# dkarpushkin/rs-pathtracing

Measured on AMD Instinct MI355X. Metric: Msamples/sec cornell_box 1920x1080x256spp at 1/2/4/8 MI355X; RMS pixel delta, higher is better.
Workload: dtype f64; 1 GPU; cornell_box.json 1920x1080 256spp depth 8; config=c2, width=1920, height=1080, spp=256, depth=8, seed=1, parallelism=single GPU, wf_slots=2

## Files before the change

rs-pathtracing_amd/csrc/pt_device.hpp:

```cpp
#pragma once
#include <hip/hip_runtime.h>

#include <cstdint>

#include "pt_lprof.hpp"
#include "pt_march.hpp"
#include "pt_torus.hpp"
#include "pt_types.hpp"

namespace pt {
namespace dev {

__device__ __forceinline__ bool stopped(const int *flag) {
    return flag && __hip_atomic_load(flag, __ATOMIC_RELAXED, __HIP_MEMORY_SCOPE_SYSTEM) != 0;
}

struct V3 {
    double x, y, z;
};
PT_HD V3 v3(double x, double y, double z) { return V3{x, y, z}; }
PT_HD V3 add(V3 a, V3 b) { return v3(a.x + b.x, a.y + b.y, a.z + b.z); }
PT_HD V3 sub(V3 a, V3 b) { return v3(a.x - b.x, a.y - b.y, a.z - b.z); }
PT_HD double dot(V3 a, V3 b) { return a.x * b.x + a.y * b.y + a.z * b.z; }
PT_HD V3 scale(V3 a, double s) { return v3(a.x * s, a.y * s, a.z * s); }
// ... 514 lines not shown
    default: {
        double g[3];
        march::shape_gradient_k<FK>(shape_params(s), p.x, p.y, p.z, g);
        n = v3(g[0], g[1], g[2]);
        break;
    }
    }
    n = normalize(n);
    V3 wn = xf_normal(s.inv, n);
    Hit h;
    h.front = dot(wn, r.d) < 0.0;
    h.n = normalize(h.front ? wn : neg(wn));
    h.p = xf_point(s.dir, p);
    return h;
}

PT_HD void hit_uv(const DShape &s, const Ray &r, double t, double *u, double *v) {
    V3 o = xf_point(s.inv, r.o);
    V3 d = xf_vector(s.inv, r.d);
    V3 p = v3(o.x + d.x * t, o.y + d.y * t, o.z + d.z * t);
    const double PI = 3.141592653589793;
    switch (s.type) {
    case SPHERE: {
        const double theta = acos(-p.y);
        const double phi = atan2(-p.z, p.x) + PI;
        *u = phi / (2.0 * PI);
        *v = theta / PI;
        return;
    }
    case RECTANGLE:
        *u = (p.x - s.p[0]) / (s.p[2] - s.p[0]);
        *v = (p.y - s.p[1]) / (s.p[3] - s.p[1]);
        return;
    case CUBE: {
        double ax = fabs(p.x), ay = fabs(p.y), az = fabs(p.z);
        double mc = fmax(fmax(ax, ay), az);
        if (mc == ax) *u = p.y, *v = p.z;
        else if (mc == ay) *u = p.x, *v = p.z;
        else if (mc == az) *u = p.x, *v = p.y;
        else *u = *v = __builtin_nan("");
        return;
    }
    case TORUS: {
        const double theta = asin(p.z / s.p[1]);
        const double phi = acos(p.z / (s.p[0] + s.p[1] * cos(theta))) + PI;
        *u = phi / (2.0 * PI);
        *v = theta / PI;
        return;
    }
    default:
        if (s.func == march::F_DUPIN || s.func == march::F_HUNTS || s.func == march::F_CUSHION) *u = p.x, *v = p.y;
        else *u = *v = 0.0;
        return;
    }
}

PT_HD int32_t sat_i32(double x) {
    if (!(x == x)) return 0;
    if (x >= 2147483647.0) return 2147483647;
    if (x <= -2147483648.0) return -2147483647 - 1;
    return (int32_t)x;
}
PT_HD uint32_t sat_u32(double x) {
    if (!(x > 0.0)) return 0u;
    if (x >= 4294967295.0) return 4294967295u;
    return (uint32_t)x;
}

PT_HD double perlin_noise(const DPerlin &P, V3 p) {
    const double fx = floor(p.x), fy = floor(p.y), fz = floor(p.z);
    const uint32_t x = (uint32_t)sat_i32(fx), y = (uint32_t)sat_i32(fy), z = (uint32_t)sat_i32(fz);
    const double u = p.x - fx, v = p.y - fy, w = p.z - fz;
    const double u2 = u * u * (3.0 - 2.0 * u);
    const double v2 = v * v * (3.0 - 2.0 * v);
    const double w2 = w * w * (3.0 - 2.0 * w);
    double acc = 0.0;
    for (int c = 0; c < 8; c++) {
        const int d0 = c >> 2, d1 = (c >> 1) & 1, d2 = c & 1;
        const int32_t k = P.perm[0][(x + (uint32_t)d0) & 255u] ^ P.perm[1][(y + (uint32_t)d1) & 255u] ^
                          P.perm[2][(z + (uint32_t)d2) & 255u];
        const double fi = (double)d0, fj = (double)d1, fk = (double)d2;
        const double dot = P.ranvec[k][0] * (u - fi) + P.ranvec[k][1] * (v - fj) + P.ranvec[k][2] * (w - fk);
        acc = acc + (fi * u2 + (double)(1 - d0) * (1.0 - u2)) * (fj * v2 + (double)(1 - d1) * (1.0 - v2)) *
                        (fk * w2 + (double)(1 - d2) * (1.0 - w2)) * dot;
    }
    return acc;
}
PT_HD double perlin_turb(const DPerlin &P, V3 p) {
    const double n = perlin_noise(P, p);
    double acc = 0.0, weight = 1.0;
    for (int i = 0; i < 7; i++) {
        acc = acc + weight * n;
        weight *= 0.5;
    }
    return fabs(acc);
}

PT_HD V3 tex_value(const Scene &sc, int node, double u, double v, V3 p) {
    const double PI = 3.141592653589793;
    for (int guard = 0; guard < 64; guard++) {
        const DTexture &t = sc.tex[node];
        switch (t.type) {
        case TEX_SOLID: return v3(t.c[0], t.c[1], t.c[2]);
        case TEX_CHECKER: {
            const double sines = sin(t.c[0] * p.x) * sin(t.c[1] * p.y) * sin(t.c[2] * p.z);
            node = sines < 0.0 ? t.odd : t.even;
            break;
        }
        case TEX_UVCHECKER: {
            const double sines = sin(v * t.c[0] * PI) * sin(u * t.c[1] * PI);
            node = sines < 0.0 ? t.odd : t.even;
            break;
        }
        case TEX_NOISE: {
            const double s = 0.5 * (1.0 + sin(t.c[0] * p.z + 10.0 * perlin_turb(sc.perlin[t.aux], p)));
            return v3(1.0 * s, 1.0 * s, 1.0 * s);
        }
        default: {
            const DImage im = sc.images[t.aux];
            const double uc = u < 0.0 ? 0.0 : (u > 1.0 ? 1.0 : u);
            const double vc = 1.0 - (v < 0.0 ? 0.0 : (v > 1.0 ? 1.0 : v));
            uint32_t x = sat_u32(uc * (double)im.width), y = sat_u32(vc * (double)im.height);
            x = x < im.width ? x : im.width - 1;
            y = y < im.height ? y : im.height - 1;
            const uint8_t *px = sc.pixels + im.offset + ((size_t)y * im.width + x) * 4;
            const double cs = 1.0 / 255.0;
            return v3((double)px[0] * cs, (double)px[1] * cs, (double)px[2] * cs);
        }
        }
    }
    return v3(__builtin_nan(""), __builtin_nan(""), __builtin_nan(""));
}

struct PhaseTimes {
    uint64_t trace, march, select, shade, passes, march_passes, finish, scatter, restart;
};
#if defined(__HIP_DEVICE_COMPILE__)
#define PT_STAMP() __builtin_amdgcn_s_memtime()
#else
#define PT_STAMP() 0ull
#endif

template <bool STATS = false>
PT_HD V3 random_in_unit_sphere(Rng &rng, double s11, Ctr *ct = nullptr) {
    for (;;) {
        PT_LP(REJECT_TRY);
        if (STATS) ct->c[C_REJECT_TRIES]++;
        double x = rng.uniform(-1.0, s11);
        double y = rng.uniform(-1.0, s11);
        double z = rng.uniform(-1.0, s11);
        if (x * x + y * y + z * z <= 1.0) return v3(x, y, z);
    }
}
PT_HD V3 reflect(V3 d, V3 n) {
    V3 b = scale(n, dot(d, n));
    return sub(d, scale(b, 2.0));
}
PT_HD V3 refract(V3 d, V3 n, double ratio) {
    double c = dot(neg(d), n);
    V3 perp = scale(add(d, scale(n, c)), ratio);
    double ps = -(sqrt(fabs(1.0 - dot(perp, perp))));
    return add(perp, scale(n, ps));
}
PT_HD V3 background(V3 d) {
    double t = 0.5 * (d.y + 1.0);
    double u = 1.0 * (1.0 - t);
    return v3(u + 0.5 * t, u + 0.7 * t, u + 1.0 * t);
}

constexpr uint32_t VAL_BIT = 0x80000000u;
template <int NW>
struct IdStack {
    uint64_t w[NW];
    int n;
    double *vb = nullptr;
    size_t vs = 0;
    PT_HD void push_val(V3 a) {
        vb[(size_t)(n * 3 + 0) * vs] = a.x;
        vb[(size_t)(n * 3 + 1) * vs] = a.y;
        vb[(size_t)(n * 3 + 2) * vs] = a.z;
        push(VAL_BIT);
    }
    PT_HD V3 val(int level) const {
        return v3(vb[(size_t)(level * 3 + 0) * vs], vb[(size_t)(level * 3 + 1) * vs], vb[(size_t)(level * 3 + 2) * vs]);
    }
    PT_HD void clear() {
#pragma unroll
        for (int i = 0; i < NW; i++) w[i] = 0;
        n = 0;
    }
    PT_HD void push(uint32_t id) {
#pragma unroll
        for (int i = NW - 1; i > 0; i--) w[i] = (w[i] << 32) | (w[i - 1] >> 32);
        w[0] = (w[0] << 32) | id;
        n++;
    }
    PT_HD uint32_t pop() {
        uint32_t id = (uint32_t)w[0];
#pragma unroll
        for (int i = 0; i < NW - 1; i++) w[i] = (w[i] >> 32) | (w[i + 1] << 32);
        w[NW - 1] >>= 32;
        n--;
        return id;
    }
};

PT_HD bool shade_decided(int who, uint32_t depth) { return depth == 0 || who < 0; }
PT_HD V3 decided_leaf(int who, const Ray &ray) { return who >= 0 ? v3(0.0, 0.0, 0.0) : background(ray.d); }

template <bool STATS = false, int FK = march::F_ANY, bool EXT = false, class Stack>
PT_HD bool shade(const Scene &sc, int who, double t, Ray &ray, uint32_t &depth, Stack &stk, Rng &rng,
                 double s11, V3 *leaf, Ctr *ct = nullptr, uint64_t *tfin = nullptr) {
    if (who < 0) {
        *leaf = background(ray.d);
        return true;
    }
    if (depth == 0) {
        *leaf = v3(0.0, 0.0, 0.0);
        return true;
    }
    const DShape &s = sc.shapes[who];
    if (STATS) ct->c[C_HITS]++;
    PT_LP(SHADE_HIT);
    Hit h = finish<FK>(s, ray, t);
    const DMaterial &m = sc.mats[s.material];
    if (tfin) *tfin = PT_STAMP();
    auto textured = [&]() {
        double u, v;
        hit_uv(s, ray, t, &u, &v);
        return tex_value(sc, m.tex, u, v, h.p);
    };
    V3 dir;
    if (m.type == LAMBERTIAN) {
        PT_LP(LAMBERT);
        if (STATS) ct->c[C_LAMBERT]++;
        V3 u = normalize(random_in_unit_sphere<STATS>(rng, s11, ct));
        dir = add(h.n, u);
        if (approx_zero(dir.x) && approx_zero(dir.y) && approx_zero(dir.z)) dir = h.n;
        if (EXT && m.tex >= 0) stk.push_val(textured());
        else stk.push((uint32_t)s.material);
    } else if (m.type == METAL) {
        PT_LP(METAL);
        if (STATS) ct->c[C_METAL]++;
        V3 rf = reflect(ray.d, h.n);
        dir = m.fuzz == 0.0 ? rf : add(rf, scale(random_in_unit_sphere<STATS>(rng, s11, ct), m.fuzz));
        if (EXT && m.tex >= 0) stk.push_val(textured());
        else stk.push((uint32_t)s.material);
    } else if (m.type == DIELECTRIC) {
        PT_LP(DIELECTRIC);
        if (STATS) ct->c[C_DIELECTRIC]++;
        double ratio = h.front ? 1.0 / m.ior : m.ior;
        double c = dot(neg(ray.d), h.n);
        double sn = sqrt(1.0 - c * c);
        bool refl = ratio * sn > 1.0;
        if (!refl) {
            double r0 = (1.0 - ratio) / (1.0 + ratio);
            r0 = r0 * r0;
            double x = 1.0 - c;
            double x5 = x * ((x * x) * (x * x));
            refl = r0 + (1.0 - r0) * x5 > rng.gen();
        }
        dir = refl ? reflect(ray.d, h.n) : refract(ray.d, h.n, ratio);
    } else {
        PT_LP(EMIT);
        if (EXT && m.type == DIFFUSE_LIGHT && m.tex >= 0) *leaf = textured();
        else *leaf = m.type == DIFFUSE_LIGHT ? v3(m.emit[0], m.emit[1], m.emit[2]) : v3(0.0, 0.0, 0.0);
        return true;
    }
    ray.o = h.p;
    ray.d = normalize(dir);
    depth--;
    return false;
}

template <bool STATS = false, bool EXT = false, class Stack>
PT_HD V3 unwind(const Scene &sc, Stack &stk, V3 c, Ctr *ct = nullptr) {
    while (stk.n > 0) {
        if (STATS) ct->c[C_UNWIND]++;
        const uint32_t id = stk.pop();
        if (EXT && (id & VAL_BIT)) {
            const V3 a = stk.val(stk.n);
            c = v3(a.x * c.x, a.y * c.y, a.z * c.z);
        } else {
            const DMaterial &m = sc.mats[id];
            c = v3(m.albedo[0] * c.x, m.albedo[1] * c.y, m.albedo[2] * c.z);
        }
    }
    return c;
}

struct MemStack {
    uint32_t *base;
    size_t stride;
    int n;
    double *vb;
    PT_HD void push_val(V3 a) {
        vb[(size_t)(n * 3 + 0) * stride] = a.x;
        vb[(size_t)(n * 3 + 1) * stride] = a.y;
        vb[(size_t)(n * 3 + 2) * stride] = a.z;
        push(VAL_BIT);
    }
    PT_HD V3 val(int level) const {
        return v3(vb[(size_t)(level * 3 + 0) * stride], vb[(size_t)(level * 3 + 1) * stride],
                  vb[(size_t)(level * 3 + 2) * stride]);
    }
    PT_HD void push(uint32_t id) {
        base[(size_t)n * stride] = id;
        n++;
    }
    PT_HD uint32_t pop() {
        n--;
        return base[(size_t)n * stride];
    }
};

template <bool EXT, class Stack>
PT_HD V3 ray_color_on(const Scene &sc, Ray ray, uint32_t depth, Rng &rng, double s11, Stack &stk) {
    V3 leaf;
    for (;;) {
        double t;
        const int who = closest<false, EXT>(sc, ray, T_MIN, __builtin_inf(), &t);
        if (shade<false, march::F_ANY, EXT>(sc, who, t, ray, depth, stk, rng, s11, &leaf)) break;
    }
    return unwind<false, EXT>(sc, stk, leaf);
}
template <int NW, bool EXT = false>
PT_HD V3 ray_color(const Scene &sc, Ray ray, uint32_t depth, Rng &rng, double s11, double *vb = nullptr,
                   size_t vs = 0) {
    IdStack<NW> stk;
    stk.clear();
    stk.vb = vb;
    stk.vs = vs;
    return ray_color_on<EXT>(sc, ray, depth, rng, s11, stk);
}
template <bool EXT = false>
PT_HD V3 ray_color_mem(const Scene &sc, Ray ray, uint32_t depth, Rng &rng, double s11, uint32_t *ids, double *vb,
                       size_t stride) {
    MemStack stk{ids, stride, 0, vb};
    return ray_color_on<EXT>(sc, ray, depth, rng, s11, stk);
}

PT_HD Ray camera_ray(const FrameParams &P, uint32_t x, uint32_t y, Rng &rng) {
    double u = rng.gen();
    double v = rng.gen();
    double sx = P.pixel_resolution * ((double)x + u);
    double sy = P.pixel_resolution * ((double)y + v);
    V3 d = v3((P.left_top[0] + P.right[0] * sx) - P.up[0] * sy, (P.left_top[1] + P.right[1] * sx) - P.up[1] * sy,
              (P.left_top[2] + P.right[2] * sx) - P.up[2] * sy);
    V3 pos = v3(P.pos[0], P.pos[1], P.pos[2]);
    Ray r;
    r.o = pos;
    r.d = normalize(sub(d, pos));
    return r;
}

constexpr int MARCH_ITERS = 2;

enum Phase : int { PH_TRACE = 0, PH_SELECT = 1, PH_MARCH = 2, PH_SHADE = 3 };


template <int NW, bool STATS = false, bool TIMING = false, int FK = march::F_ANY, bool EXT = false>
PT_HD V3 trace_pixel(const Scene &sc, const FrameParams &P, uint32_t x, uint32_t y, Ctr *ct = nullptr,
                     PhaseTimes *pt = nullptr, double *vb = nullptr, size_t vs = 0) {
    uint64_t pixel = (uint64_t)x + (uint64_t)y * P.width;
    V3 acc = v3(0.0, 0.0, 0.0);
    uint32_t s = 0;
    Rng rng{sample_key(P.seed, pixel, 0)};
    Ray ray = camera_ray(P, x, y, rng);
    uint32_t depth = P.depth;
    IdStack<NW> stk;
    stk.clear();
    stk.vb = vb;
    stk.vs = vs;
    const int nmarch = (sc.diag & 1) ? 0 : sc.nmarch;
    int phase = PH_TRACE, who = -1, km = 0, mshape = -1;
    double best = 0.0;
    V3 inv = v3(0.0, 0.0, 0.0);
    march::MarchState ms;
    march::MarchStats mst{0, 0, 0, 0};
    uint64_t ts = 0;
    for (;;) {
        if (TIMING) {
            ts = PT_STAMP();
            pt->passes++;
        }
        if (phase == PH_TRACE) {
            if (STATS) ct->c[C_BOUNCES]++;
            inv = v3(1.0 / ray.d.x, 1.0 / ray.d.y, 1.0 / ray.d.z);
            best = __builtin_inf();
            who = -1;
            closest_nomarch<STATS, EXT>(sc, ray, inv, T_MIN, &best, &who, ct);
            km = 0;
            phase = PH_SELECT;
        }
        if (TIMING) {
            uint64_t n = PT_STAMP();
            pt->trace += n - ts;
            ts = n;
// ... 83 lines not shown
```

rs-pathtracing_amd/csrc/pt_lprof.hpp:

```cpp
#pragma once
#include <hip/hip_runtime.h>

#ifdef PT_MARCH_REGIONS
namespace pt {
namespace mreg {
enum { R_ITER, R_POLY, R_PREFIX, R_HALVE, R_ADV, R_LIT, R_REFILL, R_TOTAL, R_N };
enum { P_iters, P_lin_init, P_lit_adds, P_advance_loops, P_evals, P_sir_inside, P_lin_fail_zero, P_lin_fail_q,
       P_lin_fail_tie, P_lin_fail_zone, P_N };
constexpr int G_N = 2 * R_N + 2 * P_N;
__device__ unsigned long long g_acc[G_N];
__shared__ unsigned long long t0[4][R_N], acc[4][R_N], accl[4][R_N], n0[4][R_N], pw[4][P_N], pl[4][P_N];
__device__ __forceinline__ unsigned long long now() {
    __builtin_amdgcn_sched_barrier(0);
    const unsigned long long t = __builtin_amdgcn_s_memtime();
    __builtin_amdgcn_sched_barrier(0);
    return t;
}
__device__ __forceinline__ bool leader() {
    const uint32_t lane = __builtin_amdgcn_mbcnt_hi(~0u, __builtin_amdgcn_mbcnt_lo(~0u, 0u));
    return lane == (uint32_t)__builtin_ctzll(__ballot(1));
}
__device__ __forceinline__ void begin(int r) {
    const unsigned long long m = __ballot(1);
    if (leader()) {
        t0[threadIdx.x >> 6][r] = now();
        n0[threadIdx.x >> 6][r] = __popcll(m);
    }
}
__device__ __forceinline__ void end(int r) {
    if (leader()) {
        const unsigned long long dt = now() - t0[threadIdx.x >> 6][r];
        acc[threadIdx.x >> 6][r] += dt;
        accl[threadIdx.x >> 6][r] += dt * n0[threadIdx.x >> 6][r];
    }
}
__device__ __forceinline__ void prof(int k) {
    const unsigned long long m = __ballot(1);
    if (leader()) {
        pw[threadIdx.x >> 6][k] += 1;
        pl[threadIdx.x >> 6][k] += __popcll(m);
    }
}
__device__ __forceinline__ void poly_begin() { begin(R_POLY); }
__device__ __forceinline__ void poly_end() { end(R_POLY); }
__device__ __forceinline__ void prefix_begin() { begin(R_PREFIX); }
__device__ __forceinline__ void prefix_end() { end(R_PREFIX); }
__device__ __forceinline__ void halve_begin() { begin(R_HALVE); }
__device__ __forceinline__ void halve_end() { end(R_HALVE); }
__device__ __forceinline__ void adv_begin() { begin(R_ADV); }
__device__ __forceinline__ void adv_end() { end(R_ADV); }
__device__ __forceinline__ void lit_begin() { begin(R_LIT); }
__device__ __forceinline__ void kernel_begin(unsigned long long *t_kernel) {
    if ((threadIdx.x & 63) == 0) {
        for (int k = 0; k < R_N; k++) t0[threadIdx.x >> 6][k] = acc[threadIdx.x >> 6][k] = accl[threadIdx.x >> 6][k] = 0;
        for (int k = 0; k < P_N; k++) pw[threadIdx.x >> 6][k] = pl[threadIdx.x >> 6][k] = 0;
    }
    *t_kernel = now();
}
__device__ __forceinline__ void step_end() {
    end(R_ITER);
    if (leader() && t0[threadIdx.x >> 6][R_LIT]) {
        const unsigned long long dt = now() - t0[threadIdx.x >> 6][R_LIT];
        acc[threadIdx.x >> 6][R_LIT] += dt;
        accl[threadIdx.x >> 6][R_LIT] += dt * n0[threadIdx.x >> 6][R_LIT];
        t0[threadIdx.x >> 6][R_LIT] = 0;
    }
}
__device__ __forceinline__ void kernel_end(unsigned long long t_kernel) {
    if ((threadIdx.x & 63) == 0) {
        const int w = threadIdx.x >> 6;
        acc[w][R_TOTAL] = now() - t_kernel;
        accl[w][R_TOTAL] = 0;
        for (int k = 0; k < R_N; k++) {
            atomicAdd(&g_acc[k], acc[w][k]);
            atomicAdd(&g_acc[R_N + k], accl[w][k]);
        }
        for (int k = 0; k < P_N; k++) {
            atomicAdd(&g_acc[2 * R_N + k], pw[w][k]);
            atomicAdd(&g_acc[2 * R_N + P_N + k], pl[w][k]);
        }
    }
}
}
}
#define PT_MREG(what) pt::mreg::what()
#define PT_MPROF(field) (pt::mreg::prof(pt::mreg::P_##field))
#define PT_MREG_KERNEL_BEGIN() \
    unsigned long long mreg_t_kernel_; \
    pt::mreg::kernel_begin(&mreg_t_kernel_)
#define PT_MREG_STEP_BEGIN() pt::mreg::begin(pt::mreg::R_ITER)
#define PT_MREG_STEP_END() pt::mreg::step_end()
#define PT_MREG_REFILL_BEGIN() pt::mreg::begin(pt::mreg::R_REFILL)
#define PT_MREG_REFILL_END() pt::mreg::end(pt::mreg::R_REFILL)
#define PT_MREG_KERNEL_END() pt::mreg::kernel_end(mreg_t_kernel_)
#else
#define PT_MREG_KERNEL_BEGIN() ((void)0)
#define PT_MREG_STEP_BEGIN() ((void)0)
#define PT_MREG_STEP_END() ((void)0)
#define PT_MREG_REFILL_BEGIN() ((void)0)
#define PT_MREG_REFILL_END() ((void)0)
#define PT_MREG_KERNEL_END() ((void)0)
#endif


namespace pt {
namespace lprof {
enum Point : int {
    LIVE,
    SHADE_HIT,
    LAMBERT,
    REJECT_TRY,
    METAL,
    DIELECTRIC,
    EMIT,
    ENDED,
    TRACE,
    ULIST_SHAPE,
    RECT_ROWS,
    UBOX_PASS,
    BVH_NODE,
    BVH_ENTER,
    BVH_LEAF,
    PRE_SLAB,
    PRE_JOB,
    ANY_END,
    MISS_END,
    STORE,
    N_POINTS
};
}
}

#if defined(PT_LANE_PROF)
namespace pt {
namespace lprof {
static __device__ unsigned long long g_counts[2 * N_POINTS];
static __shared__ unsigned long long s_pass[N_POINTS], s_lanes[N_POINTS];
__device__ __forceinline__ void hit(int k) {
    const unsigned long long m = __ballot(1);
    const uint32_t lane = __builtin_amdgcn_mbcnt_hi(~0u, __builtin_amdgcn_mbcnt_lo(~0u, 0u));
    if (lane == (uint32_t)__builtin_ctzll(m)) {
        atomicAdd(&s_pass[k], 1ull);
        atomicAdd(&s_lanes[k], (unsigned long long)__popcll(m));
    }
}
__device__ __forceinline__ void begin_kernel() {
    if (threadIdx.x < N_POINTS) s_pass[threadIdx.x] = s_lanes[threadIdx.x] = 0;
    __syncthreads();
}
__device__ __forceinline__ void end_kernel() {
    __syncthreads();
    if (threadIdx.x < N_POINTS) {
        atomicAdd(&g_counts[threadIdx.x], s_pass[threadIdx.x]);
        atomicAdd(&g_counts[N_POINTS + threadIdx.x], s_lanes[threadIdx.x]);
    }
}
}
}
#endif
#if defined(PT_LANE_PROF) && defined(__HIP_DEVICE_COMPILE__)
#define PT_LP(k) pt::lprof::hit(pt::lprof::k)
#define PT_LP_BEGIN() pt::lprof::begin_kernel()
#define PT_LP_END() pt::lprof::end_kernel()
#else
#define PT_LP(k) ((void)0)
#define PT_LP_BEGIN() ((void)0)
#define PT_LP_END() ((void)0)
#endif
```

rs-pathtracing_amd/csrc/pt_wave.hip:

```cpp
#include <hip/hip_runtime.h>

#include <cstdio>
#include <cstdlib>
#include <vector>

#include "pt_lprof.hpp"

#include "pt_device.hpp"
#include "pt_kernel.hpp"
#include "pt_plan.hpp"

namespace pt {

using dev::MemStack;
using dev::Ray;
using dev::V3;

constexpr uint32_t WHO_MASK = (1u << 25) - 1u;
__host__ __device__ __forceinline__ uint32_t pack_who(int who, uint32_t count) {
    return (uint32_t)(who + 1) | (count << 25);
}
__host__ __device__ __forceinline__ int unpack_who(uint32_t w) { return (int)(w & WHO_MASK) - 1; }

struct PathSoA {
    char *base;
    size_t cap;
    static constexpr size_t BYTES = PATH_BYTES;
    static constexpr uint32_t BLK = 64, BLK_BYTES = (uint32_t)BYTES * BLK;
    enum F8 : int { OX, OY, OZ, DX, DY, DZ, T, RNG };
    enum F4 : int { WHO, SID };
    __host__ __device__ double *d8(uint32_t k) const {
        return (double *)(base + (size_t)(k / BLK) * BLK_BYTES) + (k % BLK);
    }
    __host__ __device__ uint32_t *d4(uint32_t k) const {
        return (uint32_t *)(base + (size_t)(k / BLK) * BLK_BYTES + 8 * 8 * BLK) + (k % BLK);
    }
    __host__ __device__ double &t(uint32_t k) const { return d8(k)[T * BLK]; }
    __host__ __device__ uint32_t &who(uint32_t k) const { return d4(k)[WHO * BLK]; }
};

struct WfView {
    PathSoA in, out;
    uint32_t *ids;
    double *att;
    double *leaf;
    uint8_t *status;
    uint32_t *list, *mq;
    double2 *jo;
    uint32_t *cnt;
    double *acc;
    uint32_t cap;
    uint32_t npix;
    uint32_t s0, ns;
    uint32_t tile0;
};

struct WfArgs {
    dev::Scene sc;
    FrameParams P;
    WfView v;
};

template <class T>
__device__ __forceinline__ const T &kargs(const T *p) {
    typedef const __attribute__((address_space(4))) T *cptr;
    cptr q = (cptr)p;
    asm volatile("" : "+s"(q));
    return *(const T *)q;
}

__device__ __forceinline__ uint32_t lane_id() {
    return __builtin_amdgcn_mbcnt_hi(~0u, __builtin_amdgcn_mbcnt_lo(~0u, 0u));
}

constexpr int UB = 4;
template <bool EXT>
__device__ __forceinline__ V3 unwind_mem(const dev::Scene &sc, MemStack &stk, V3 c) {
    if (EXT) return dev::unwind<false, true>(sc, stk, c);
    while (stk.n > 0) {
        const int m = stk.n < UB ? stk.n : UB;
        uint32_t id[UB];
#pragma unroll
        for (int j = 0; j < UB; j++) id[j] = j < m ? stk.base[(size_t)(stk.n - 1 - j) * stk.stride] : 0u;
        double ax[UB], ay[UB], az[UB];
#pragma unroll
        for (int j = 0; j < UB; j++) {
            const DMaterial &mt = sc.mats[id[j]];
            ax[j] = j < m ? mt.albedo[0] : 1.0;
            ay[j] = j < m ? mt.albedo[1] : 1.0;
            az[j] = j < m ? mt.albedo[2] : 1.0;
        }
#pragma unroll
        for (int j = 0; j < UB; j++)
            if (j < m) c = dev::v3(ax[j] * c.x, ay[j] * c.y, az[j] * c.z);
        stk.n -= m;
    }
    return c;
}

__device__ __forceinline__ void end_path(const WfView &v, uint32_t id, const MemStack &stk, V3 leaf) {
    typedef double d2v __attribute__((ext_vector_type(2)));
    d2v *rec = (d2v *)(v.leaf + (size_t)id * 4);
    __builtin_nontemporal_store((d2v){leaf.x, leaf.y}, rec);
    __builtin_nontemporal_store((d2v){leaf.z, __builtin_bit_cast(double, (uint64_t)(uint32_t)stk.n)}, rec + 1);
}

template <typename T>
__device__ __forceinline__ void st_path(T *p, T x) {
    __builtin_nontemporal_store(x, p);
}
template <typename T>
__device__ __forceinline__ T ld_path(const T *p) {
    return *p;
}
__device__ __forceinline__ void store_path(const PathSoA &S, uint32_t k, uint32_t id, const Ray &ray, double best,
                                           int who, uint64_t rng, uint32_t count) {
    double *a = S.d8(k);
    uint32_t *b = S.d4(k);
    constexpr uint32_t B = PathSoA::BLK;
    st_path(a + PathSoA::OX * B, ray.o.x);
    st_path(a + PathSoA::OY * B, ray.o.y);
    st_path(a + PathSoA::OZ * B, ray.o.z);
    st_path(a + PathSoA::DX * B, ray.d.x);
    st_path(a + PathSoA::DY * B, ray.d.y);
    st_path(a + PathSoA::DZ * B, ray.d.z);
    st_path(a + PathSoA::T * B, best);
    st_path(b + PathSoA::WHO * B, pack_who(who, count));
    st_path((uint64_t *)a + PathSoA::RNG * B, (uint64_t)rng);
    st_path(b + PathSoA::SID * B, id);
}
__device__ __forceinline__ void load_path(const PathSoA &S, uint32_t p, uint32_t *id, Ray *ray, uint64_t *rng,
                                          uint32_t depth_it, uint32_t *depth, uint32_t *count, int *who,
                                          double *best) {
    const double *a = S.d8(p);
    const uint32_t *b = S.d4(p);
    constexpr uint32_t B = PathSoA::BLK;
    *id = ld_path(b + PathSoA::SID * B);
    ray->o = dev::v3(ld_path(a + PathSoA::OX * B), ld_path(a + PathSoA::OY * B), ld_path(a + PathSoA::OZ * B));
    ray->d = dev::v3(ld_path(a + PathSoA::DX * B), ld_path(a + PathSoA::DY * B), ld_path(a + PathSoA::DZ * B));
    *rng = ld_path((const uint64_t *)a + PathSoA::RNG * B);
    const uint32_t w = ld_path(b + PathSoA::WHO * B);
    *who = unpack_who(w);
    *count = w >> 25;
    *depth = depth_it;
    *best = ld_path(a + PathSoA::T * B);
}

static_assert(plan::PACKED_COUNT_DEPTH == MAX_REG_DEPTH, "the DEEP builds start where the register stacks end");
__device__ __forceinline__ uint32_t *deep_count(const WfView &v, uint32_t depth, uint32_t id) {
    return v.ids + (size_t)depth * v.cap + id;
}

__device__ __forceinline__ void slot_pixel(const FrameParams &P, const WfView &v, uint32_t id, uint32_t *x,
                                           uint32_t *y, uint32_t *s_local, uint32_t *pix_local) {
    const uint32_t within = id % v.npix;
    *s_local = id / v.npix;
    *pix_local = within;
    const uint32_t ti = v.tile0 + within / (TILE * TILE);
    const uint32_t th = within % (TILE * TILE);
    const uint32_t k = dev::tile_position(P.rank + ti * P.world, P.tiles_x, P.world);
    const uint32_t tx = k % P.tiles_x, ty = k / P.tiles_x;
    const uint32_t w = th >> 6, l = th & 63;
    *x = tx * TILE + (((w & 1u) << 3) | (l & 7u));
    *y = ty * TILE + (((w >> 1) << 3) | (l >> 3));
}

constexpr int WF_PREDICT = 4;

template <bool FIRST, int WAVES, int FK = march::F_ANY, bool EXT = false, bool BIGBVH = false, bool SPLIT = false,
          bool DEEP = false>
__global__ __launch_bounds__(256, WAVES) void wf_bounce(const WfArgs *__restrict__ A, int it,
                                                        unsigned long long *diag = nullptr) {
    uint32_t count;
    {
        const WfArgs &a = kargs(A);
        const WfView &v = a.v;
        count = FIRST ? (v.cnt[3] ? 0u : v.ns * v.npix) : v.cnt[it * 4 + 0];
        if (a.P.stop && blockIdx.x == 0 && threadIdx.x == 0 && v.cnt[3]) dev::note_stop(a.sc.guard, count > 0);
    }
    const uint32_t stride = gridDim.x * blockDim.x;
    const bool DIAG = PT_WAVE_DIAG && diag;
    unsigned long long dsec[7] = {0, 0, 0, 0, 0, 0, 0}, tst = 0;
    PT_LP_BEGIN();
#define PT_BSTAMP(k)                                                \
    if (DIAG) {                                                     \
        __builtin_amdgcn_s_waitcnt(0);                              \
        const unsigned long long n_ = __builtin_amdgcn_s_memtime(); \
        dsec[k] += n_ - tst;                                        \
        tst = n_;                                                   \
    }
    for (uint32_t base = blockIdx.x * blockDim.x; base < count; base += stride) {
        if (DIAG) tst = __builtin_amdgcn_s_memtime();
        const WfArgs &a = kargs(A);
        const dev::Scene &sc = a.sc;
        const FrameParams &P = a.P;
        const WfView &v = a.v;
        const uint32_t i = base + threadIdx.x;
        bool live = i < count;
        uint32_t id = 0;
        Ray ray;
        dev::Rng rng{0};
        uint32_t depth = 0;
        MemStack stk{v.ids, (size_t)v.cap, 0, nullptr};
        int who = -1;
        double best = 0.0;
        if (live) {
            if (FIRST) {
                id = i;
                uint32_t x, y, sl, pl;
                slot_pixel(P, v, id, &x, &y, &sl, &pl);
                if (x >= P.width || y >= P.height || sl >= v.ns) {
                    live = false;
                } else {
                    rng.s = dev::sample_key(P.seed, (uint64_t)x + (uint64_t)y * P.width, v.s0 + sl);
                    ray = dev::camera_ray(P, x, y, rng);
                    depth = P.depth;
                    stk.base = v.ids + id;
                    if (EXT) stk.vb = v.att + id;
                }
            } else {
                const uint32_t p = v.list[i];
                PT_BSTAMP(0)
                uint32_t count;
                load_path(v.in, p, &id, &ray, &rng.s, P.depth + 1u - (uint32_t)it, &depth, &count, &who, &best);
                stk.base = v.ids + id;
                stk.n = DEEP ? (int)*deep_count(v, P.depth, id) : (int)count;
                if (EXT) stk.vb = v.att + id;
                PT_BSTAMP(1)
            }
        }
        bool need_march = false, long_job = false;
        V3 jo_o = dev::v3(0.0, 0.0, 0.0), jo_d = jo_o;
        double jo_st = 0.0, jo_en = 0.0;
        if (live) {
            PT_LP(LIVE);
            if (!FIRST) {
                V3 leaf;
                const bool ended = dev::shade<false, FK, EXT>(kargs(A).sc, who, best, ray, depth, stk, rng, P.s11, &leaf);
                PT_BSTAMP(2)
                if (ended) {
                    PT_LP(ENDED);
                    end_path(v, id, stk, leaf);
                    live = false;
                    PT_BSTAMP(3)
                }
            }
        }
        if (live && SPLIT) {
            best = __builtin_inf();
            who = -1;
        } else if (live) {
            PT_LP(TRACE);
            const V3 inv = dev::v3(1.0 / ray.d.x, 1.0 / ray.d.y, 1.0 / ray.d.z);
            best = __builtin_inf();
            who = -1;
            const bool any = depth == 0;
            dev::closest_nomarch<false, EXT, BIGBVH>(kargs(A).sc, ray, inv, T_MIN, &best, &who, nullptr, any);
            PT_BSTAMP(4)
            for (int k = 0; k < sc.nmarch && !need_march && !(any && who >= 0); k++) {
                const int s = dev::uniform_index(dev::uniform_load(&sc.march[k]));
                const DBox bx = dev::uniform_box(&sc.boxes[s]);
                if (!dev::slab(bx.lo, bx.hi, ray, inv, T_MIN, best)) continue;
                PT_LP(PRE_SLAB);
                const DShape S = dev::uniform_shape(&sc.shapes[s]);
                jo_o = dev::xf_point(S.inv, ray.o);
                jo_d = dev::xf_vector(S.inv, ray.d);
                need_march = march::shape_bound_k<FK>(dev::shape_params(S), jo_o.x, jo_o.y, jo_o.z, jo_d.x, jo_d.y,
                                                      jo_d.z, &jo_st, &jo_en);
            }
            PT_BSTAMP(5)
            if (!need_march && dev::shade_decided(who, depth)) {
                if (any) PT_LP(ANY_END);
                else PT_LP(MISS_END);
                end_path(v, id, stk, dev::decided_leaf(who, ray));
                live = false;
            }
        }
        const uint32_t wbase = base + (threadIdx.x & ~63u);
        const uint64_t keep = __ballot(live);
        const uint32_t k = wbase + (uint32_t)__popcll(keep & ((1ull << (threadIdx.x & 63)) - 1ull));
        if (i < count && (threadIdx.x & 63) >= (uint32_t)__popcll(keep)) v.status[i] = 0u;
        if (need_march && v.jo) {
            PT_LP(PRE_JOB);
            typedef double d2v __attribute__((ext_vector_type(2)));
            d2v *j = (d2v *)(v.jo + (size_t)k * 4);
            __builtin_nontemporal_store((d2v){jo_o.x, jo_o.y}, j + 0);
            __builtin_nontemporal_store((d2v){jo_o.z, jo_d.x}, j + 1);
            __builtin_nontemporal_store((d2v){jo_d.y, jo_d.z}, j + 2);
            __builtin_nontemporal_store((d2v){jo_st, jo_en}, j + 3);
            const march::FParams F = dev::shape_params(dev::uniform_shape(&sc.shapes[dev::uniform_index(
                dev::uniform_load(&sc.march[0]))]));
            const V3 o = jo_o, d = jo_d;
            const double st = jo_st, en = jo_en;
            long_job = march::shape_f_k<FK>(F, o.x + d.x * st, o.y + d.y * st, o.z + d.z * st) < 0.0;
            const double dt = (en - st) * (1.0 / WF_PREDICT);
#pragma unroll
            for (int q = 0; q < WF_PREDICT; q++) {
                const double tq = st + dt * (q + 0.5);
                long_job = long_job || march::shape_f_k<FK>(F, o.x + d.x * tq, o.y + d.y * tq, o.z + d.z * tq) < 0.0;
            }
        }
        if (i < count) PT_LP(STORE);
        if (i < count && live) {
            store_path(v.out, k, id, ray, best, who, rng.s, DEEP ? 0u : (uint32_t)stk.n);
            if (DEEP) *deep_count(v, P.depth, id) = (uint32_t)stk.n;
            v.status[k] = live ? (need_march ? (long_job ? 7u : 3u) : 1u) : 0u;
        }
        PT_BSTAMP(6)
    }
#undef PT_BSTAMP
    PT_LP_END();
    if (DIAG && (threadIdx.x & 63) == 0)
        for (int k = 0; k < 7; k++) atomicAdd(&diag[36 + k], dsec[k]);
}


__device__ __forceinline__ void cp_bits(uint4 q, uint32_t *live, uint32_t *march, uint32_t *lng) {
    const uint32_t w[4] = {q.x, q.y, q.z, q.w};
    uint32_t l = 0, m = 0, g = 0;
#pragma unroll
    for (int k = 0; k < 4; k++) {
        l += __popc(w[k] & 0x01010101u);
        m += __popc(w[k] & 0x02020202u);
        g += __popc(w[k] & 0x04040404u);
    }
    *live = l;
    *march = m;
    *lng = g;
}

__device__ __forceinline__ uint32_t block_exscan(uint32_t x, uint32_t *total, uint32_t *lds ) {
    const uint32_t lane = threadIdx.x & 63, wv = threadIdx.x >> 6;
    uint32_t inc = x;
#pragma unroll
    for (int o = 1; o < 64; o <<= 1) {
        const uint32_t y = __shfl_up(inc, o, 64);
        if (lane >= (uint32_t)o) inc += y;
    }
    if (lane == 63) lds[wv] = inc;
    __syncthreads();
    uint32_t before = 0, tot = 0;
#pragma unroll
    for (int k = 0; k < 4; k++) {
        if ((uint32_t)k < wv) before += lds[k];
        tot += lds[k];
    }
    __syncthreads();
    *total = tot;
    return before + inc - x;
}

__device__ __forceinline__ uint4 cp_load(const uint8_t *__restrict__ st, uint32_t tile, uint32_t n) {
    const uint32_t b = tile * CP_TILE + threadIdx.x * CP_ITEMS;
    if (b >= n) return make_uint4(0u, 0u, 0u, 0u);
    uint4 q = reinterpret_cast<const uint4 *>(st + (size_t)tile * CP_TILE)[threadIdx.x];
    if (n - b < (uint32_t)CP_ITEMS) {
        const uint32_t k = n - b;
        uint32_t w[4] = {q.x, q.y, q.z, q.w};
#pragma unroll
        for (int j = 0; j < 4; j++) {
            const uint32_t keep = k >= 4u * (j + 1) ? 4u : (k > 4u * j ? k - 4u * j : 0u);
            w[j] &= keep >= 4u ? 0xffffffffu : ((1u << (8u * keep)) - 1u);
        }
        q = make_uint4(w[0], w[1], w[2], w[3]);
    }
    return q;
}

struct CpLayout {
    uint32_t per, stride;
    __host__ __device__ static CpLayout of(uint32_t tiles) {
        const uint32_t per = (tiles + CP_BLOCK - 1) / CP_BLOCK;
        return CpLayout{per ? per : 1u, (per ? per : 1u) * CP_BLOCK};
    }
    __device__ uint32_t at(uint32_t b) const { return (b % per) * CP_BLOCK + b / per; }
};

constexpr uint32_t CP_GRID = 2048;
__device__ __forceinline__ uint32_t cp_n(const uint32_t *n_dev, uint32_t n_host) { return n_dev ? *n_dev : n_host; }

__global__ __launch_bounds__(256) void cp_count(const uint8_t *__restrict__ st, uint32_t *__restrict__ blk, CpLayout L,
                                                const uint32_t *__restrict__ n_dev, uint32_t n_host) {
    __shared__ uint32_t lds[12];
    const uint32_t n = cp_n(n_dev, n_host), nt = (n + CP_TILE - 1) / CP_TILE;
    for (uint32_t tb = blockIdx.x; tb < nt; tb += gridDim.x) {
        const uint4 q = cp_load(st, tb, n);
        uint32_t l, m, g, tl, tg, ts;
        cp_bits(q, &l, &m, &g);
        block_exscan(l, &tl, lds);
        block_exscan(g, &tg, lds + 4);
        block_exscan(m - g, &ts, lds + 8);
        if (threadIdx.x == 0) {
            const uint32_t k = L.at(tb);
            blk[k] = tl;
            blk[L.stride + k] = tg;
            blk[2 * L.stride + k] = ts;
        }
    }
}

constexpr int SCAN_RUN = 48;
__global__ __launch_bounds__(256) void cp_scan(uint32_t *__restrict__ blk, uint32_t nblk_max, CpLayout L,
                                               const uint32_t *__restrict__ n_dev, uint32_t n_host,
                                               uint32_t *__restrict__ n_live, uint32_t *__restrict__ n_march,
                                               uint32_t *__restrict__ n_long) {
    __shared__ uint32_t lds[12];
    const uint32_t nt = (cp_n(n_dev, n_host) + CP_TILE - 1) / CP_TILE;
    const uint32_t nblk = nt < nblk_max ? nt : nblk_max;
    const uint32_t per = L.per;
    const uint32_t b0 = threadIdx.x * per;
    const uint32_t nj = b0 >= nblk ? 0u : (nblk - b0 < per ? nblk - b0 : per);
    uint32_t *bl = blk + threadIdx.x, *bg = bl + L.stride, *bs = bg + L.stride;
    uint32_t sl = 0, sg = 0, ss = 0, tl, tg, ts;
    if (per <= (uint32_t)SCAN_RUN) {
        uint32_t rl[SCAN_RUN], rg[SCAN_RUN], rs[SCAN_RUN];
#pragma unroll
        for (int j = 0; j < SCAN_RUN; j++) {
            const bool ok = (uint32_t)j < nj;
            rl[j] = ok ? bl[j * CP_BLOCK] : 0u;
            rg[j] = ok ? bg[j * CP_BLOCK] : 0u;
            rs[j] = ok ? bs[j * CP_BLOCK] : 0u;
        }
#pragma unroll
        for (int j = 0; j < SCAN_RUN; j++) sl += rl[j], sg += rg[j], ss += rs[j];
        uint32_t cl = block_exscan(sl, &tl, lds), cg = block_exscan(sg, &tg, lds + 4), cs = block_exscan(ss, &ts, lds + 8);
#pragma unroll
        for (int j = 0; j < SCAN_RUN; j++) {
            if ((uint32_t)j < nj) {
                bl[j * CP_BLOCK] = cl;
                bg[j * CP_BLOCK] = cg;
                bs[j * CP_BLOCK] = cs;
            }
            cl += rl[j];
            cg += rg[j];
            cs += rs[j];
        }
    } else {
#pragma unroll 8
        for (uint32_t j = 0; j < nj; j++) {
            sl += bl[j * CP_BLOCK];
            sg += bg[j * CP_BLOCK];
            ss += bs[j * CP_BLOCK];
        }
        uint32_t cl = block_exscan(sl, &tl, lds), cg = block_exscan(sg, &tg, lds + 4), cs = block_exscan(ss, &ts, lds + 8);
#pragma unroll 8
        for (uint32_t j = 0; j < nj; j++) {
            const uint32_t l = bl[j * CP_BLOCK], g = bg[j * CP_BLOCK], h = bs[j * CP_BLOCK];
            bl[j * CP_BLOCK] = cl;
            bg[j * CP_BLOCK] = cg;
            bs[j * CP_BLOCK] = cs;
            cl += l;
            cg += g;
            cs += h;
        }
    }
    if (threadIdx.x == 0) {
        *n_live = tl;
        *n_march = tg + ts;
        *n_long = tg;
    }
}
// ... 801 lines not shown
```

Measured before the change: 2212 Msamples/s.

## Precompute sphere rejection counts ahead in a wave-cooperative work queue

Before shading, each wave loads the RNG states of the next several grid-stride trips into LDS. It then runs the unit-sphere rejection loop cooperatively, with lanes pulling new items from a shared cursor, so the divergent rejection tries are balanced across lanes. The per-item rejection count is stored in LDS, and shading skips the RNG state forward by that count before its final accepted draw. This removes warp divergence from rejection sampling, at the cost of extra RNG-state loads, LDS use (8 KB+ per block), a cap of 15 rejections, and restructured grid-stride loops.

```diff
diff --git a/rs-pathtracing_amd/csrc/pt_device.hpp b/rs-pathtracing_amd/csrc/pt_device.hpp
--- a/rs-pathtracing_amd/csrc/pt_device.hpp
+++ b/rs-pathtracing_amd/csrc/pt_device.hpp
@@ -690,6 +690,44 @@
         if (x * x + y * y + z * z <= 1.0) return v3(x, y, z);
     }
 }
+constexpr uint32_t DRAW_CAP = 15;
+PT_HD bool sphere_try_accepts(Rng &rng, double s11) {
+    double x = rng.uniform(-1.0, s11);
+    double y = rng.uniform(-1.0, s11);
+    double z = rng.uniform(-1.0, s11);
+    return x * x + y * y + z * z <= 1.0;
+}
+PT_HD uint32_t sphere_rejects(Rng rng, double s11, uint32_t cap = DRAW_CAP) {
+    uint32_t k = 0;
+    while (k < cap && !sphere_try_accepts(rng, s11)) k++;
+    return k;
+}
+template <bool STATS = false>
+PT_HD V3 sphere_point_after(Rng &rng, double s11, uint32_t k, Ctr *ct = nullptr) {
+    rng.s += (uint64_t)(3u * k) * GAMMA;
+    if (STATS) ct->c[C_REJECT_TRIES] += k;
+    return random_in_unit_sphere<STATS>(rng, s11, ct);
+}
+template <class Packed = uint64_t>
+PT_HD Packed draw_ahead_lane(const uint64_t *st, size_t stride, uint32_t n, double s11) {
+    Packed packed = 0;
+    uint32_t j = 0, c = 0;
+    Rng r{n ? st[0] : 0ull};
+    while (j < n) {
+        PT_LP(DRAW_TRY);
+        const bool acc = sphere_try_accepts(r, s11);
+        if (!acc) c++;
+        if (acc || c == DRAW_CAP) {
+            packed |= (Packed)c << (4u * j);
+            j++;
+            c = 0;
+            if (j < n) r.s = st[(size_t)j * stride];
+        }
+    }
+    return packed;
+}
+PT_HD uint32_t draw_ahead_count(uint64_t packed, uint32_t j) { return (uint32_t)(packed >> (4u * j)) & 15u; }
+
 PT_HD V3 reflect(V3 d, V3 n) {
     V3 b = scale(n, dot(d, n));
     return sub(d, scale(b, 2.0));
@@ -748,7 +786,7 @@
 
 template <bool STATS = false, int FK = march::F_ANY, bool EXT = false, class Stack>
 PT_HD bool shade(const Scene &sc, int who, double t, Ray &ray, uint32_t &depth, Stack &stk, Rng &rng,
-                 double s11, V3 *leaf, Ctr *ct = nullptr, uint64_t *tfin = nullptr) {
+                 double s11, V3 *leaf, Ctr *ct = nullptr, uint64_t *tfin = nullptr, int ahead = -1) {
     if (who < 0) {
         *leaf = background(ray.d);
         return true;
@@ -772,7 +810,7 @@
     if (m.type == LAMBERTIAN) {
         PT_LP(LAMBERT);
         if (STATS) ct->c[C_LAMBERT]++;
-        V3 u = normalize(random_in_unit_sphere<STATS>(rng, s11, ct));
+        V3 u = normalize(sphere_point_after<STATS>(rng, s11, ahead < 0 ? 0u : (uint32_t)ahead, ct));
         dir = add(h.n, u);
         if (approx_zero(dir.x) && approx_zero(dir.y) && approx_zero(dir.z)) dir = h.n;
         if (EXT && m.tex >= 0) stk.push_val(textured());
@@ -781,7 +819,9 @@
         PT_LP(METAL);
         if (STATS) ct->c[C_METAL]++;
         V3 rf = reflect(ray.d, h.n);
-        dir = m.fuzz == 0.0 ? rf : add(rf, scale(random_in_unit_sphere<STATS>(rng, s11, ct), m.fuzz));
+        dir = m.fuzz == 0.0
+                  ? rf
+                  : add(rf, scale(sphere_point_after<STATS>(rng, s11, ahead < 0 ? 0u : (uint32_t)ahead, ct), m.fuzz));
         if (EXT && m.tex >= 0) stk.push_val(textured());
         else stk.push((uint32_t)s.material);
     } else if (m.type == DIELECTRIC) {
diff --git a/rs-pathtracing_amd/csrc/pt_lprof.hpp b/rs-pathtracing_amd/csrc/pt_lprof.hpp
--- a/rs-pathtracing_amd/csrc/pt_lprof.hpp
+++ b/rs-pathtracing_amd/csrc/pt_lprof.hpp
@@ -110,6 +110,7 @@
     SHADE_HIT,
     LAMBERT,
     REJECT_TRY,
+    DRAW_TRY,
     METAL,
     DIELECTRIC,
     EMIT,
diff --git a/rs-pathtracing_amd/csrc/pt_wave.hip b/rs-pathtracing_amd/csrc/pt_wave.hip
--- a/rs-pathtracing_amd/csrc/pt_wave.hip
+++ b/rs-pathtracing_amd/csrc/pt_wave.hip
@@ -2,6 +2,7 @@
 
 #include <cstdio>
 #include <cstdlib>
+#include <type_traits>
 #include <vector>
 
 #include "pt_lprof.hpp"
@@ -167,6 +168,17 @@
 
 constexpr int WF_PREDICT = 4;
 
+#ifndef WF_DRAW_AHEAD
+#define WF_DRAW_AHEAD 8
+#endif
+#ifndef WF_DRAW_MIN
+#define WF_DRAW_MIN 3
+#endif
+#ifndef WF_DRAW_SHARED
+#define WF_DRAW_SHARED 1
+#endif
+static_assert(WF_DRAW_AHEAD >= 0 && WF_DRAW_AHEAD <= 16, "the counts of a round are 4 bits each in 64");
+
 template <bool FIRST, int WAVES, int FK = march::F_ANY, bool EXT = false, bool BIGBVH = false, bool SPLIT = false,
           bool DEEP = false>
 __global__ __launch_bounds__(256, WAVES) void wf_bounce(const WfArgs *__restrict__ A, int it,
@@ -189,124 +201,199 @@
         dsec[k] += n_ - tst;                                        \
         tst = n_;                                                   \
     }
-    for (uint32_t base = blockIdx.x * blockDim.x; base < count; base += stride) {
-        if (DIAG) tst = __builtin_amdgcn_s_memtime();
-        const WfArgs &a = kargs(A);
-        const dev::Scene &sc = a.sc;
-        const FrameParams &P = a.P;
-        const WfView &v = a.v;
-        const uint32_t i = base + threadIdx.x;
-        bool live = i < count;
-        uint32_t id = 0;
-        Ray ray;
-        dev::Rng rng{0};
-        uint32_t depth = 0;
-        MemStack stk{v.ids, (size_t)v.cap, 0, nullptr};
-        int who = -1;
-        double best = 0.0;
-        if (live) {
-            if (FIRST) {
-                id = i;
-                uint32_t x, y, sl, pl;
-                slot_pixel(P, v, id, &x, &y, &sl, &pl);
-                if (x >= P.width || y >= P.height || sl >= v.ns) {
+    constexpr uint32_t RT = FIRST || !WF_DRAW_AHEAD ? 1u : (uint32_t)WF_DRAW_AHEAD;
+    constexpr bool AHEAD = RT > 1;
+    typedef typename std::conditional<(RT > 8), uint64_t, uint32_t>::type ahead_t;
+    __shared__ uint64_t draw_st[AHEAD ? RT * 256 : 1];
+#if WF_DRAW_SHARED
+    __shared__ uint8_t draw_cn[AHEAD ? RT * 256 : 1];
+#endif
+    for (uint32_t rbase = blockIdx.x * blockDim.x; rbase < count; rbase += RT * stride) {
+        ahead_t ahead = 0;
+        const bool drawn = AHEAD && count - rbase > (WF_DRAW_MIN - 1u) * stride;
+        if (drawn) {
+            const WfArgs &a = kargs(A);
+            const WfView &v = a.v;
+            uint64_t *col = draw_st + (threadIdx.x & ~63u) * RT + (threadIdx.x & 63u);
+            uint32_t p[RT], n = 0;
+#pragma unroll
+            for (uint32_t j = 0; j < RT; j++) {
+                const uint32_t i = rbase + j * stride + threadIdx.x;
+                p[j] = v.list[i < count ? i : count - 1u];
+                n += i < count ? 1u : 0u;
+            }
+            uint64_t s[RT];
+#pragma unroll
+            for (uint32_t j = 0; j < RT; j++)
+                s[j] = ld_path((const uint64_t *)v.in.d8(p[j]) + PathSoA::RNG * PathSoA::BLK);
+#pragma unroll
+            for (uint32_t j = 0; j < RT; j++) col[j * 64] = s[j];
+#if WF_DRAW_SHARED
+            uint32_t E = 0;
+#pragma unroll
+            for (uint32_t j = 0; j < RT; j++)
+                E += (uint32_t)__popcll(__ballot(rbase + j * stride + threadIdx.x < count));
+            const uint32_t lane = threadIdx.x & 63u;
+            const uint64_t *wst = draw_st + (threadIdx.x & ~63u) * RT;
+            uint8_t *wcn = draw_cn + (threadIdx.x & ~63u) * RT;
+            __builtin_amdgcn_fence(__ATOMIC_RELEASE, "wavefront");
+            __builtin_amdgcn_wave_barrier();
+            __builtin_amdgcn_fence(__ATOMIC_ACQUIRE, "wavefront");
+            uint32_t item = lane, cursor = 64u, c = 0;
+            bool has = item < E;
+            dev::Rng r{has ? wst[item] : 0ull};
+            const double s11 = a.P.s11;
+            while (has) {
+                PT_LP(DRAW_TRY);
+                const bool acc = dev::sphere_try_accepts(r, s11);
+                if (!acc) c++;
+                const bool fin = acc || c == dev::DRAW_CAP;
+                const uint64_t fm = __ballot(fin);
+                if (fin) {
+                    wcn[item] = (uint8_t)c;
+                    item = cursor + (uint32_t)__popcll(fm & ((1ull << lane) - 1ull));
+                    c = 0;
+                    has = item < E;
+                    if (has) r.s = wst[item];
+                }
+                cursor += (uint32_t)__popcll(fm);
+            }
+            __builtin_amdgcn_fence(__ATOMIC_RELEASE, "wavefront");
+            __builtin_amdgcn_wave_barrier();
+            __builtin_amdgcn_fence(__ATOMIC_ACQUIRE, "wavefront");
+            (void)n;
+#else
+            ahead = dev::draw_ahead_lane<ahead_t>(col, 64, n, a.P.s11);
+#endif
+        }
+#pragma unroll 1
+        for (uint32_t trip = 0; trip < RT; trip++) {
+            const uint32_t base = rbase + trip * stride;
+            if (base >= count) break;
+            if (DIAG) tst = __builtin_amdgcn_s_memtime();
+            const WfArgs &a = kargs(A);
+            const dev::Scene &sc = a.sc;
+            const FrameParams &P = a.P;
+            const WfView &v = a.v;
+            const uint32_t i = base + threadIdx.x;
+            bool live = i < count;
+#if WF_DRAW_SHARED
+            if (drawn) ahead = draw_cn[(threadIdx.x & ~63u) * RT + trip * 64u + (threadIdx.x & 63u)];
+#endif
+            uint32_t id = 0;
+            Ray ray;
+            dev::Rng rng{0};
+            uint32_t depth = 0;
+            MemStack stk{v.ids, (size_t)v.cap, 0, nullptr};
+            int who = -1;
+            double best = 0.0;
+            if (live) {
+                if (FIRST) {
+                    id = i;
+                    uint32_t x, y, sl, pl;
+                    slot_pixel(P, v, id, &x, &y, &sl, &pl);
+                    if (x >= P.width || y >= P.height || sl >= v.ns) {
+                        live = false;
+                    } else {
+                        rng.s = dev::sample_key(P.seed, (uint64_t)x + (uint64_t)y * P.width, v.s0 + sl);
+                        ray = dev::camera_ray(P, x, y, rng);
+                        depth = P.depth;
+                        stk.base = v.ids + id;
+                        if (EXT) stk.vb = v.att + id;
+                    }
+                } else {
+                    const uint32_t p = v.list[i];
+                    PT_BSTAMP(0)
+                    uint32_t count;
+                    load_path(v.in, p, &id, &ray, &rng.s, P.depth + 1u - (uint32_t)it, &depth, &count, &who, &best);
+                    stk.base = v.ids + id;
+                    stk.n = DEEP ? (int)*deep_count(v, P.depth, id) : (int)count;
+                    if (EXT) stk.vb = v.att + id;
+                    PT_BSTAMP(1)
+                }
+            }
+            bool need_march = false, long_job = false;
+            V3 jo_o = dev::v3(0.0, 0.0, 0.0), jo_d = jo_o;
+            double jo_st = 0.0, jo_en = 0.0;
+            if (live) {
+                PT_LP(LIVE);
+                if (!FIRST) {
+                    V3 leaf;
+                    const bool ended = dev::shade<false, FK, EXT>(kargs(A).sc, who, best, ray, depth, stk, rng, P.s11, &leaf,
+                                                                  nullptr, nullptr,
+                                                                  drawn ? (int)(ahead & 15u) : -1);
+                    PT_BSTAMP(2)
+                    if (ended) {
+                        PT_LP(ENDED);
+                        end_path(v, id, stk, leaf);
+                        live = false;
+                        PT_BSTAMP(3)
+                    }
+                }
+            }
+            if (live && SPLIT) {
+                best = __builtin_inf();
+                who = -1;
+            } else if (live) {
+                PT_LP(TRACE);
+                const V3 inv = dev::v3(1.0 / ray.d.x, 1.0 / ray.d.y, 1.0 / ray.d.z);
+                best = __builtin_inf();
+                who = -1;
+                const bool any = depth == 0;
+                dev::closest_nomarch<false, EXT, BIGBVH>(kargs(A).sc, ray, inv, T_MIN, &best, &who, nullptr, any);
+                PT_BSTAMP(4)
+                for (int k = 0; k < sc.nmarch && !need_march && !(any && who >= 0); k++) {
+                    const int s = dev::uniform_index(dev::uniform_load(&sc.march[k]));
+                    const DBox bx = dev::uniform_box(&sc.boxes[s]);
+                    if (!dev::slab(bx.lo, bx.hi, ray, inv, T_MIN, best)) continue;
+                    PT_LP(PRE_SLAB);
+                    const DShape S = dev::uniform_shape(&sc.shapes[s]);
+                    jo_o = dev::xf_point(S.inv, ray.o);
+                    jo_d = dev::xf_vector(S.inv, ray.d);
+                    need_march = march::shape_bound_k<FK>(dev::shape_params(S), jo_o.x, jo_o.y, jo_o.z, jo_d.x, jo_d.y,
+                                                          jo_d.z, &jo_st, &jo_en);
+                }
+                PT_BSTAMP(5)
+                if (!need_march && dev::shade_decided(who, depth)) {
+                    if (any) PT_LP(ANY_END);
+                    else PT_LP(MISS_END);
+                    end_path(v, id, stk, dev::decided_leaf(who, ray));
                     live = false;
-                } else {
-                    rng.s = dev::sample_key(P.seed, (uint64_t)x + (uint64_t)y * P.width, v.s0 + sl);
-                    ray = dev::camera_ray(P, x, y, rng);
-                    depth = P.depth;
-                    stk.base = v.ids + id;
-                    if (EXT) stk.vb = v.att + id;
                 }
-            } else {
-                const uint32_t p = v.list[i];
-                PT_BSTAMP(0)
-                uint32_t count;
-                load_path(v.in, p, &id, &ray, &rng.s, P.depth + 1u - (uint32_t)it, &depth, &count, &who, &best);
-                stk.base = v.ids + id;
-                stk.n = DEEP ? (int)*deep_count(v, P.depth, id) : (int)count;
-                if (EXT) stk.vb = v.att + id;
-                PT_BSTAMP(1)
-            }
-        }
-        bool need_march = false, long_job = false;
-        V3 jo_o = dev::v3(0.0, 0.0, 0.0), jo_d = jo_o;
-        double jo_st = 0.0, jo_en = 0.0;
-        if (live) {
-            PT_LP(LIVE);
-            if (!FIRST) {
-                V3 leaf;
-                const bool ended = dev::shade<false, FK, EXT>(kargs(A).sc, who, best, ray, depth, stk, rng, P.s11, &leaf);
-                PT_BSTAMP(2)
-                if (ended) {
-                    PT_LP(ENDED);
-                    end_path(v, id, stk, leaf);
-                    live = false;
-                    PT_BSTAMP(3)
+            }
+            const uint32_t wbase = base + (threadIdx.x & ~63u);
+            const uint64_t keep = __ballot(live);
+            const uint32_t k = wbase + (uint32_t)__popcll(keep & ((1ull << (threadIdx.x & 63)) - 1ull));
+            if (i < count && (threadIdx.x & 63) >= (uint32_t)__popcll(keep)) v.status[i] = 0u;
+            if (need_march && v.jo) {
+                PT_LP(PRE_JOB);
+                typedef double d2v __attribute__((ext_vector_type(2)));
+                d2v *j = (d2v *)(v.jo + (size_t)k * 4);
+                __builtin_nontemporal_store((d2v){jo_o.x, jo_o.y}, j + 0);
+                __builtin_nontemporal_store((d2v){jo_o.z, jo_d.x}, j + 1);
+                __builtin_nontemporal_store((d2v){jo_d.y, jo_d.z}, j + 2);
+                __builtin_nontemporal_store((d2v){jo_st, jo_en}, j + 3);
+                const march::FParams F = dev::shape_params(dev::uniform_shape(&sc.shapes[dev::uniform_index(
+                    dev::uniform_load(&sc.march[0]))]));
+                const V3 o = jo_o, d = jo_d;
+                const double st = jo_st, en = jo_en;
+                long_job = march::shape_f_k<FK>(F, o.x + d.x * st, o.y + d.y * st, o.z + d.z * st) < 0.0;
+                const double dt = (en - st) * (1.0 / WF_PREDICT);
+#pragma unroll
+                for (int q = 0; q < WF_PREDICT; q++) {
+                    const double tq = st + dt * (q + 0.5);
+                    long_job = long_job || march::shape_f_k<FK>(F, o.x + d.x * tq, o.y + d.y * tq, o.z + d.z * tq) < 0.0;
                 }
             }
-        }
-        if (live && SPLIT) {
-            best = __builtin_inf();
-            who = -1;
-        } else if (live) {
-            PT_LP(TRACE);
-            const V3 inv = dev::v3(1.0 / ray.d.x, 1.0 / ray.d.y, 1.0 / ray.d.z);
-            best = __builtin_inf();
-            who = -1;
-            const bool any = depth == 0;
-            dev::closest_nomarch<false, EXT, BIGBVH>(kargs(A).sc, ray, inv, T_MIN, &best, &who, nullptr, any);
-            PT_BSTAMP(4)
-            for (int k = 0; k < sc.nmarch && !need_march && !(any && who >= 0); k++) {
-                const int s = dev::uniform_index(dev::uniform_load(&sc.march[k]));
-                const DBox bx = dev::uniform_box(&sc.boxes[s]);
-                if (!dev::slab(bx.lo, bx.hi, ray, inv, T_MIN, best)) continue;
-                PT_LP(PRE_SLAB);
-                const DShape S = dev::uniform_shape(&sc.shapes[s]);
-                jo_o = dev::xf_point(S.inv, ray.o);
-                jo_d = dev::xf_vector(S.inv, ray.d);
-                need_march = march::shape_bound_k<FK>(dev::shape_params(S), jo_o.x, jo_o.y, jo_o.z, jo_d.x, jo_d.y,
-                                                      jo_d.z, &jo_st, &jo_en);
-            }
-            PT_BSTAMP(5)
-            if (!need_march && dev::shade_decided(who, depth)) {
-                if (any) PT_LP(ANY_END);
-                else PT_LP(MISS_END);
-                end_path(v, id, stk, dev::decided_leaf(who, ray));
-                live = false;
-            }
-        }
-        const uint32_t wbase = base + (threadIdx.x & ~63u);
-        const uint64_t keep = __ballot(live);
-        const uint32_t k = wbase + (uint32_t)__popcll(keep & ((1ull << (threadIdx.x & 63)) - 1ull));
-        if (i < count && (threadIdx.x & 63) >= (uint32_t)__popcll(keep)) v.status[i] = 0u;
-        if (need_march && v.jo) {
-            PT_LP(PRE_JOB);
-            typedef double d2v __attribute__((ext_vector_type(2)));
-            d2v *j = (d2v *)(v.jo + (size_t)k * 4);
-            __builtin_nontemporal_store((d2v){jo_o.x, jo_o.y}, j + 0);
-            __builtin_nontemporal_store((d2v){jo_o.z, jo_d.x}, j + 1);
-            __builtin_nontemporal_store((d2v){jo_d.y, jo_d.z}, j + 2);
-            __builtin_nontemporal_store((d2v){jo_st, jo_en}, j + 3);
-            const march::FParams F = dev::shape_params(dev::uniform_shape(&sc.shapes[dev::uniform_index(
-                dev::uniform_load(&sc.march[0]))]));
-            const V3 o = jo_o, d = jo_d;
-            const double st = jo_st, en = jo_en;
-            long_job = march::shape_f_k<FK>(F, o.x + d.x * st, o.y + d.y * st, o.z + d.z * st) < 0.0;
-            const double dt = (en - st) * (1.0 / WF_PREDICT);
-#pragma unroll
-            for (int q = 0; q < WF_PREDICT; q++) {
-                const double tq = st + dt * (q + 0.5);
-                long_job = long_job || march::shape_f_k<FK>(F, o.x + d.x * tq, o.y + d.y * tq, o.z + d.z * tq) < 0.0;
-            }
-        }
-        if (i < count) PT_LP(STORE);
-        if (i < count && live) {
-            store_path(v.out, k, id, ray, best, who, rng.s, DEEP ? 0u : (uint32_t)stk.n);
-            if (DEEP) *deep_count(v, P.depth, id) = (uint32_t)stk.n;
-            v.status[k] = live ? (need_march ? (long_job ? 7u : 3u) : 1u) : 0u;
-        }
-        PT_BSTAMP(6)
+            if (i < count) PT_LP(STORE);
+            if (i < count && live) {
+                store_path(v.out, k, id, ray, best, who, rng.s, DEEP ? 0u : (uint32_t)stk.n);
+                if (DEEP) *deep_count(v, P.depth, id) = (uint32_t)stk.n;
+                v.status[k] = live ? (need_march ? (long_job ? 7u : 3u) : 1u) : 0u;
+            }
+            PT_BSTAMP(6)
+            ahead >>= 4;
+        }
     }
 #undef PT_BSTAMP
     PT_LP_END();
```

Result: no change. 2229 Msamples/s (median of 6 runs) (+0.7%).
